# fgcallari/skeres

Hardware: AMD Instinct MI355X
Metric: LM iterations/sec (higher is better)
Workload: dtype f64

## Files before the change

### skeres_amd/csrc/chol_kernels.hip

```cpp
#include <hip/hip_runtime.h>
#include <algorithm>
#include <atomic>
#include <chrono>
#include <hip/hip_ext.h>
#include <math.h>
#include <stdlib.h>
#include <string.h>
#include <memory>
#include "chol_kernels.hpp"
#include "device_table.hpp"

namespace sk {

typedef double d4 __attribute__((ext_vector_type(4)));

constexpr int gemm_lds_doubles(int kBKT, int kTM, int kTN) { return 2 * (kTM + kTN) * (kBKT + 2); }
#define SK_GEMM_LDS(kBKT, kTM, kTN) __shared__ __attribute__((aligned(16))) double sh[gemm_lds_doubles(kBKT, kTM, kTN)];
template <int kMode, int kShape, int kBKT, int kPF, int kTM, int kTN>
__device__ __forceinline__ void gemm_nt_f64_body(double* shp, double* C, long ldc, const double* A, long lda, const double* B, long ldb, int K,
                                                 int tiles_m, int skip, int main_t = 0x7fffffff, int jump_t = 0, int main_n = 0x7fffffff,
                                                 int jump_n = 0, int block_id = -1, int* first_column_done = nullptr, int count_cols = 1,
                                                 int* diag_done = nullptr) {
  constexpr int mode = kMode;
  constexpr int kLdT = kBKT + 2;
// ... 85 lines not shown
  if (kPF == 2) { SK_LOAD_STAGE(1, (nk > 1 ? 1 : 0) * kBKT) }
  SK_STORE_STAGE(0, 0)
  __syncthreads();
#define SK_LOAD_STAGE_X(set, kbase) SK_LOAD_STAGE(set, kbase)
#define SK_STORE_STAGE_X(set, buf) SK_STORE_STAGE(set, buf)
#define SK_KSTEP(kt, SETL, SETS)                                                                   \
  {                                                                                                \
    const int buf = (kt) & 1;                                                                      \
    const int knext = ((kt) + kPF < nk ? (kt) + kPF : nk - 1) * kBKT;                              \
    SK_LOAD_STAGE_X(SETL, knext)                                                                   \
    const double* sa = &shp[buf * kShBuf + (wr * (kTM / 2) + l15) * kLdT + l4];                               \
    const double* sb = &shp[buf * kShBuf + (kTM + wc * (kTN / 2) + l15) * kLdT + l4];                         \
    _Pragma("unroll") for (int kk = 0; kk < kBKT / 4; ++kk) {                                      \
      double a[kMT], b[kNT];                                                                       \
      _Pragma("unroll") for (int m = 0; m < kMT; ++m) a[m] = sa[m * 16 * kLdT + kk * 4];           \
      _Pragma("unroll") for (int m = 0; m < kNT; ++m) b[m] = sb[m * 16 * kLdT + kk * 4];           \
      _Pragma("unroll") for (int mt = 0; mt < kMT; ++mt)                                           \
        _Pragma("unroll") for (int nt = 0; nt < kNT; ++nt)                                         \
          acc[mt][nt] = __builtin_amdgcn_mfma_f64_16x16x4f64(a[mt], b[nt], acc[mt][nt], 0, 0, 0);  \
    }                                                                                              \
    SK_STORE_STAGE_X(SETS, buf ^ 1)                                                                \
    __syncthreads();                                                                               \
  }
  if (kPF == 1) {
    for (int kt = 0; kt < nk; ++kt) SK_KSTEP(kt, 0, 0)
  } else {
    for (int kt = 0; kt < nk; kt += 2) {
      SK_KSTEP(kt, 0, 1)
      SK_KSTEP(kt + 1, 1, 0)
    }
  }
#undef SK_KSTEP
#undef SK_LOAD_STAGE_X
#undef SK_STORE_STAGE_X
  (void)ra1; (void)rb1;
#undef SK_LOAD_STAGE
#undef SK_STORE_STAGE
  const double sgn = mode == 0 ? -1.0 : 1.0;
  if (kShape == 2 && first_column_done && first_column) {
#pragma unroll
    for (int mt = 0; mt < kMT; ++mt)
#pragma unroll
      for (int nt = 0; nt < kNT; ++nt)
#pragma unroll
        for (int i = 0; i < 4; ++i)
          __hip_atomic_store(&Cg[(long)(crow + mt * 16 + 4 * i) * ldc + ccol + nt * 16], sgn * acc[mt][nt][i], __ATOMIC_RELAXED, __HIP_MEMORY_SCOPE_AGENT);
    asm volatile("s_waitcnt vmcnt(0) lgkmcnt(0)" ::: "memory");
    __syncthreads();
    if (threadIdx.x == 0) {
      __hip_atomic_fetch_add(first_column_done, 1, __ATOMIC_RELAXED, __HIP_MEMORY_SCOPE_AGENT);
      if (diag_done && diag_tile) __hip_atomic_fetch_add(diag_done, 16 / (128 / kTM), __ATOMIC_RELAXED, __HIP_MEMORY_SCOPE_AGENT);
    }
    return;
  }
#pragma unroll
  for (int mt = 0; mt < kMT; ++mt)
#pragma unroll
    for (int nt = 0; nt < kNT; ++nt)
#pragma unroll
      for (int i = 0; i < 4; ++i)
        Cg[(long)(crow + mt * 16 + 4 * i) * ldc + ccol + nt * 16] = sgn * acc[mt][nt][i];
}

__global__ __launch_bounds__(256, 2) void syrk_trailing_f64_kernel(double* C, long ldc, const double* A, long lda, int K, int tile_off, int main_t,
                                                                   int jump_t) {
  SK_GEMM_LDS(16, 128, 128)
  gemm_nt_f64_body<0, 1, 16, 1, 128, 128>(sh, C, ldc, A, lda, A, lda, K, 0, tile_off, main_t, jump_t);
}
__global__ __launch_bounds__(256, 2) void syrk_trailing_thin_f64_kernel(double* C, long ldc, const double* A, long lda, int K, int tiles_m, int main_t,
                                                                        int jump_t, int main_n, int jump_n, int* first_column_done, int count_cols, int* diag_done) {
  SK_GEMM_LDS(16, 32, 128)
  gemm_nt_f64_body<0, 2, 16, 2, 32, 128>(sh, C, ldc, A, lda, A, lda, K, tiles_m, 0, main_t, jump_t, main_n, jump_n, -1, first_column_done, count_cols, diag_done);
}
struct ThinSyrkArgs { double* C; long ldc; const double* A; long lda; int K, tiles_m, main_t, jump_t, main_n, jump_n; int* first_column_done; int grid; };
struct ThinSyrkPair { ThinSyrkArgs f[2]; };
__global__ __launch_bounds__(256, 2) void syrk_trailing_thin_pair_f64_kernel(ThinSyrkPair pair) {
  const ThinSyrkArgs& p = pair.f[blockIdx.y];
  if ((int)blockIdx.x >= p.grid) return;
  SK_GEMM_LDS(16, 32, 128)
  gemm_nt_f64_body<0, 2, 16, 2, 32, 128>(sh, p.C, p.ldc, p.A, p.lda, p.A, p.lda, p.K, p.tiles_m, 0, p.main_t, p.jump_t, p.main_n, p.jump_n, -1, p.first_column_done, 1, nullptr);
}
__global__ __launch_bounds__(256, 2) void syrk_gram_f64_kernel(double* C, long ldc, size_t slab_stride, const double* A, long lda, int K) {
  SK_GEMM_LDS(16, 128, 128)
  gemm_nt_f64_body<1, 1, 16, 1, 128, 128>(sh, C + (size_t)blockIdx.y * slab_stride, ldc, A + (size_t)blockIdx.y * K, lda, A + (size_t)blockIdx.y * K, lda, K, 0, 0);
}
__global__ __launch_bounds__(256) void gram_reduce_kernel(double* __restrict__ H, const double* __restrict__ slabs, size_t slab_stride, long ld,
                                                          int nslabs) {
  const int b = blockIdx.x;
  int r = (int)((sqrt(8.0 * (double)b + 1.0) - 1.0) * 0.5);
  while ((r + 1) * (r + 2) / 2 <= b) ++r;
  while (r * (r + 1) / 2 > b) --r;
  const int ti = r, tj = b - r * (r + 1) / 2;
  for (int e = threadIdx.x; e < 128 * 128; e += 256) {
    const size_t off = (size_t)(ti * 128 + (e >> 7)) * ld + tj * 128 + (e & 127);
    double s = 0.0;
    for (int c = 0; c < nslabs; ++c) s += slabs[(size_t)c * slab_stride + off];
    H[off] = s;
  }
}
__global__ __launch_bounds__(256, 2) void gemm_update_f64_kernel(double* C, long ldc, const double* A, long lda, const double* B,
                                                                 long ldb, int K, int tiles_m, int skip, int main_t, int jump_t) {
  __builtin_amdgcn_s_setprio(2);
  SK_GEMM_LDS(16, 64, 128)
  gemm_nt_f64_body<0, 0, 16, 2, 64, 128>(sh, C, ldc, A, lda, B, ldb, K, tiles_m, skip, main_t, jump_t);
}
__global__ __launch_bounds__(256, 2) void gemm_update_thin_f64_kernel(double* C, long ldc, const double* A, long lda, const double* B,
                                                                      long ldb, int K, int tiles_m, int skip, int main_t, int jump_t) {
  __builtin_amdgcn_s_setprio(2);
  SK_GEMM_LDS(16, 32, 128)
  gemm_nt_f64_body<0, 0, 16, 2, 32, 128>(sh, C, ldc, A, lda, B, ldb, K, tiles_m, skip, main_t, jump_t);
}
__global__ __launch_bounds__(256, 2) void trsm_gemm_thin_f64_kernel(double* C, long ldc, const double* A, long lda, const double* Linv,
                                                                    int tiles_m, int main_t, int jump_t) {
  __builtin_amdgcn_s_setprio(2);
  SK_GEMM_LDS(16, 32, 128)
  gemm_nt_f64_body<1, 0, 16, 2, 32, 128>(sh, C, ldc, A, lda, Linv, 128, 128, tiles_m, 0, main_t, jump_t);
}
__global__ __launch_bounds__(256, 1) void gemm_diag_f64_kernel(double* C, long ldc, const double* A, long lda, int K) {
  __builtin_amdgcn_s_setprio(3);
  SK_GEMM_LDS(32, 64, 64)
  gemm_nt_f64_body<0, 0, 32, 2, 64, 64>(sh, C, ldc, A, lda, A, lda, K, 2, 4);
}
__global__ __launch_bounds__(256, 2) void trsm_gemm_f64_kernel(double* C, long ldc, const double* A, long lda, const double* Linv,
                                                               int tiles_m, int main_t, int jump_t) {
  __builtin_amdgcn_s_setprio(2);
  SK_GEMM_LDS(16, 64, 128)
  gemm_nt_f64_body<1, 0, 16, 2, 64, 128>(sh, C, ldc, A, lda, Linv, 128, 128, tiles_m, 0, main_t, jump_t);
}

static constexpr int kB = 32, kBs = 33;
static constexpr int kBlk = kB * kBs;
__device__ __forceinline__ int blk_off(int bi, int bj) { return (bi * (bi + 1) / 2 + bj) * kBlk; }
__device__ __forceinline__ int inv_off(int bi, int bj) { return (10 + bi * (bi - 1) / 2 + bj) * kBlk; }

__device__ __forceinline__ double fast_rsqrt(double x) {
  double y = __builtin_amdgcn_rsq(x);
  double h = 0.5 * x;
  y = y * (1.5 - h * y * y);
  y = y * (1.5 - h * y * y);
  return y;
}
__device__ __forceinline__ double fast_rcp(double x) {
  const double y = __builtin_amdgcn_rcp(x);
  const double e = __builtin_fma(-x, y, 1.0);
  const double q = __builtin_fma(e, e, e);
  return __builtin_fma(y, q, y);
}
__device__ __forceinline__ double lane_bcast(double x, int src) {
  const int lo = __builtin_amdgcn_readlane(__double2loint(x), src);
  const int hi = __builtin_amdgcn_readlane(__double2hiint(x), src);
  return __hiloint2double(hi, lo);
}

__device__ __forceinline__ bool wave_potrf32(const double* D, double* colbuf, double (&a)[32], int lane) {
  const int row = lane & 31;
  const bool unit = lane >= 32;
#pragma unroll
  for (int c = 0; c < 32; ++c) {
    const double d = D[row * kBs + c];
    a[c] = unit ? (c == row ? 1.0 : 0.0) : d;
  }
  colbuf[lane] = a[0];
  typedef __attribute__((address_space(3))) const double* lds_cdp;
  unsigned cb_base = (unsigned)(unsigned long)(lds_cdp)colbuf;
  asm volatile("" : "+v"(cb_base));
  const lds_cdp cb3 = (lds_cdp)(unsigned long)cb_base;
  double cbp[32], cbn[32];
  double m_prev = 0.0, d_prev = 1.0;
  int dv_lo = 0, dv_hi = 0x3ff00000;
  int sgn = 0;
#define SK_PIN(x) asm volatile("" : "+v"(x));
#ifndef SK_PROBE_VARIANT
#define SK_PROBE_VARIANT 0
#endif
#define SK_FILL(k)                                                                                  \
  if (j >= 1 && SK_PROBE_VARIANT != 1) {                                                                                     \
    _Pragma("unroll") for (int c = j + 1 + ((k) * (31 - j) + 4) / 5; c < j + 1 + (((k) + 1) * (31 - j) + 4) / 5; ++c)  \
      a[c] = __builtin_fma(-m_prev, cbp[c], a[c]);                                                  \
  }
#pragma unroll
  for (int j = 0; j < 32; ++j) {
    {
      const lds_cdp cbj = cb3 + (j % 3) * 64;
#pragma unroll
      for (int c = j + 2; c < 32; ++c) cbn[c] = SK_PROBE_VARIANT == 2 ? a[c] * 0.5 : cbj[c];
    }
    const int d_lo = __builtin_amdgcn_readlane(__double2loint(a[j]), j), d_hi = __builtin_amdgcn_readlane(__double2hiint(a[j]), j);
    const double d = __hiloint2double(d_hi, d_lo);
    const double y = __builtin_amdgcn_rcp(d);
    const double l1 = lane_bcast(a[j], j + 1 < 32 ? j + 1 : j);
    const double m0 = a[j] * y;
    __builtin_amdgcn_sched_barrier(0);
    sgn |= d_hi;
    asm volatile("" : "+s"(sgn));
    asm volatile("v_writelane_b32 %0, %1, %2" : "+v"(dv_lo) : "s"(d_lo), "n"(j));
    asm volatile("v_writelane_b32 %0, %1, %2" : "+v"(dv_hi) : "s"(d_hi), "n"(j));
    SK_FILL(0)
    __builtin_amdgcn_sched_barrier(0);
    const double e = __builtin_fma(-d, y, 1.0);
    __builtin_amdgcn_sched_barrier(0);
    SK_FILL(1)
    __builtin_amdgcn_sched_barrier(0);
    const double q = __builtin_fma(e, e, e);
    __builtin_amdgcn_sched_barrier(0);
    SK_FILL(2)
    __builtin_amdgcn_sched_barrier(0);
    const double m = __builtin_fma(m0, q, m0);
    __builtin_amdgcn_sched_barrier(0);
    SK_FILL(3)
    __builtin_amdgcn_sched_barrier(0);
    if (j + 1 < 32) {
      a[j + 1] = __builtin_fma(-m, l1, a[j + 1]);
      colbuf[((j + 1) % 3) * 64 + lane] = a[j + 1];
    }
    __builtin_amdgcn_sched_barrier(0);
    SK_FILL(4)
    __builtin_amdgcn_sched_barrier(0);
    m_prev = m;
    d_prev = d;
#pragma unroll
    for (int c = j + 2; c < 32; ++c) cbp[c] = cbn[c];
  }
#undef SK_FILL
#undef SK_PIN
  {
    const double r = fast_rsqrt(__hiloint2double(dv_hi, dv_lo));
#pragma unroll
    for (int c = 0; c < 32; ++c) a[c] = a[c] * lane_bcast(r, c);
  }
  return sgn >= 0 && d_prev > 0.0;
}

template <bool kPlainB>
__device__ __forceinline__ void block_mma32(d4 (&acc)[2][2], const double* P, const double* Q, int lane) {
  const int l15 = lane & 15, l4 = lane >> 4;
#pragma unroll
  for (int kk = 0; kk < 8; ++kk) {
    const int k = kk * 4 + l4;
    double a[2], b[2];
#pragma unroll
    for (int m = 0; m < 2; ++m) {
      a[m] = P[(m * 16 + l15) * kBs + k];
      b[m] = kPlainB ? Q[k * kBs + m * 16 + l15] : Q[(m * 16 + l15) * kBs + k];
    }
#pragma unroll
    for (int mt = 0; mt < 2; ++mt)
#pragma unroll
      for (int nt = 0; nt < 2; ++nt)
        acc[mt][nt] = __builtin_amdgcn_mfma_f64_16x16x4f64(a[mt], b[nt], acc[mt][nt], 0, 0, 0);
  }
}
__device__ __forceinline__ void quad_mma16(d4& acc, const double* P, const double* Q, int qi, int qj, int lane, bool fresh) {
  const int l15 = lane & 15, l4 = lane >> 4;
  d4 a0 = fresh ? (d4){0.0, 0.0, 0.0, 0.0} : acc, a1 = (d4){0.0, 0.0, 0.0, 0.0};
#pragma unroll
  for (int kk = 0; kk < 8; kk += 2) {
    const int k = kk * 4 + l4;
    a0 = __builtin_amdgcn_mfma_f64_16x16x4f64(P[(qi * 16 + l15) * kBs + k], Q[(qj * 16 + l15) * kBs + k], a0, 0, 0, 0);
    a1 = __builtin_amdgcn_mfma_f64_16x16x4f64(P[(qi * 16 + l15) * kBs + k + 4], Q[(qj * 16 + l15) * kBs + k + 4], a1, 0, 0, 0);
  }
  acc = a0 + a1;
}
__device__ __forceinline__ void quad_store16(double* dst, const d4& acc, int qi, int qj, int lane, double sgn) {
  const int l15 = lane & 15, l4 = lane >> 4;
#pragma unroll
  for (int i = 0; i < 4; ++i) dst[(qi * 16 + l4 + 4 * i) * kBs + qj * 16 + l15] = sgn * acc[i];
}
__device__ __forceinline__ void quad_load16(d4& acc, const double* src, int qi, int qj, int lane, double sgn) {
  const int l15 = lane & 15, l4 = lane >> 4;
#pragma unroll
  for (int i = 0; i < 4; ++i) acc[i] = sgn * src[(qi * 16 + l4 + 4 * i) * kBs + qj * 16 + l15];
}
__device__ __forceinline__ void block_zero32(d4 (&acc)[2][2]) {
#pragma unroll
  for (int mt = 0; mt < 2; ++mt)
#pragma unroll
    for (int nt = 0; nt < 2; ++nt) acc[mt][nt] = (d4){0.0, 0.0, 0.0, 0.0};
}
__device__ __forceinline__ void block_store32(double* dst, const d4 (&acc)[2][2], int lane, double sgn) {
  const int l15 = lane & 15, l4 = lane >> 4;
#pragma unroll
  for (int mt = 0; mt < 2; ++mt)
#pragma unroll
    for (int nt = 0; nt < 2; ++nt)
#pragma unroll
      for (int i = 0; i < 4; ++i) dst[(mt * 16 + l4 + 4 * i) * kBs + nt * 16 + l15] = sgn * acc[mt][nt][i];
}
__device__ __forceinline__ void block_load32(d4 (&acc)[2][2], const double* src, int lane, double sgn) {
  const int l15 = lane & 15, l4 = lane >> 4;
#pragma unroll
  for (int mt = 0; mt < 2; ++mt)
#pragma unroll
    for (int nt = 0; nt < 2; ++nt)
#pragma unroll
      for (int i = 0; i < 4; ++i) acc[mt][nt][i] = sgn * src[(mt * 16 + l4 + 4 * i) * kBs + nt * 16 + l15];
}
__device__ __forceinline__ void block_update32(double* Cb, const double* P, const double* Q, int lane) {
  d4 acc[2][2];
  block_load32(acc, Cb, lane, -1.0);
  block_mma32<false>(acc, P, Q, lane);
  block_store32(Cb, acc, lane, -1.0);
}
__device__ __forceinline__ void block_to_global(double* dst, unsigned step2, unsigned goff, const double* src, int loff) {
#pragma unroll
  for (int i = 0; i < 16; ++i) dst[goff + i * step2] = src[loff + i * 2 * kBs];
}
__device__ __forceinline__ void block_neg_left_mul32(double* dst, const double* W, int lane) {
  d4 acc[2][2];
  block_zero32(acc);
  block_mma32<true>(acc, W, dst, lane);
  block_store32(dst, acc, lane, -1.0);
}

#ifdef SK_POTRF_STAMPS
__device__ long long g_potrf_stamps[4][16], g_potrf_clk[4][16];
#define SK_STAMP(i) if (lane == 0) { g_potrf_stamps[wave][i] = wall_clock64(); g_potrf_clk[wave][i] = clock64(); }
#else
#define SK_STAMP(i)
#endif

__device__ __forceinline__ void info_raise(int* info, int v) { (void)__hip_atomic_fetch_max(info, v, __ATOMIC_RELAXED, __HIP_MEMORY_SCOPE_AGENT); }

__device__ __forceinline__ void potrf128_body(double* lds_in, double* __restrict__ A, long ld, double* __restrict__ Linv, int* info) {
  double* lds = lds_in;
  int tid = threadIdx.x;
  asm volatile("" : "+v"(tid), "+s"(ld));
  double* T = lds;
  double* E = lds + 16 * kBlk;
  double* colbuf = lds + 18 * kBlk;
  volatile int* flags = reinterpret_cast<volatile int*>(colbuf + 192);
  const int t = tid, lane = t & 63, wave = __builtin_amdgcn_readfirstlane(t >> 6);
  __builtin_amdgcn_s_setprio(3);
  SK_STAMP(0)
  {
    double v0[4];
#pragma unroll
    for (int i = 0; i < 4; ++i) {
      const int e = t + 256 * i;
      v0[i] = A[(long)(e >> 5) * ld + (e & 31)];
    }
    if (wave == 0) {
#pragma unroll
      for (int i = 0; i < 4; ++i) { const int e = t + 256 * i; T[blk_off(0, 0) + (e >> 5) * kBs + (e & 31)] = v0[i]; }
      if (t < 4) flags[t] = 0;
      __syncthreads();
    } else {
      double v[3][16];
      const int first = 3 * (wave - 1) + 1;
      const long lo = (long)(lane >> 5) * ld + (lane & 31);
#pragma unroll
      for (int k = 0; k < 3; ++k) {
        const int idx = first + k, bi = idx >= 6 ? 3 : (idx >= 3 ? 2 : 1), bj = idx - bi * (bi + 1) / 2;
        const double* Ab = A + ((long)bi * kB * ld + bj * kB) + lo;
#pragma unroll
        for (int i = 0; i < 16; ++i) v[k][i] = Ab[(long)(2 * i) * ld];
      }
#pragma unroll
      for (int i = 0; i < 4; ++i) { const int e = t + 256 * i; T[blk_off(0, 0) + (e >> 5) * kBs + (e & 31)] = v0[i]; }
      __syncthreads();
      const int ll = (lane >> 5) * kBs + (lane & 31);
#pragma unroll
      for (int k = 0; k < 3; ++k) {
        const int idx = first + k, bi = idx >= 6 ? 3 : (idx >= 3 ? 2 : 1), bj = idx - bi * (bi + 1) / 2;
#pragma unroll
        for (int i = 0; i < 16; ++i) T[blk_off(bi, bj) + ll + 2 * i * kBs] = v[k][i];
      }
    }
  }
  SK_STAMP(1)
  const unsigned uld = (unsigned)ld;
  const unsigned go_a = (unsigned)(lane >> 5) * uld + (lane & 31), go_i = (unsigned)(lane >> 5) * 128u + (lane & 31);
  const int lo_w = (lane >> 5) * kBs + (lane & 31);
#define SK_L(bi, bj) (T + blk_off(bi, bj))
#define SK_V(bi, bj) (T + inv_off(bi, bj))
#define SK_GA(bi, bj) (A + ((long)(bi) * kB * ld + (bj) * kB))
#define SK_GI(bi, bj) (Linv + ((bi) * kB * 128 + (bj) * kB))
#define SK_PANEL_ROW(jb, bi)                                                                    \
  {                                                                                             \
    d4 acc[2][2];                                                                               \
    block_zero32(acc);                                                                          \
    block_mma32<false>(acc, SK_L(bi, jb), SK_L(jb, jb), lane);                                  \
    block_store32(SK_L(bi, jb), acc, lane, 1.0);   \
  }
#define SK_CRITICAL_B(jb)                                                                        \
  {                                                                                              \
    d4 xq;                                                                                       \
    quad_mma16(xq, SK_L((jb) + 1, jb), SK_L(jb, jb), qi, qj, lane, true);                        \
    __syncthreads();                                         \
    quad_store16(SK_L((jb) + 1, jb), xq, qi, qj, lane, 1.0);                                     \
    __syncthreads();                                                 \
    d4 uq;                                                                                       \
    quad_load16(uq, SK_L((jb) + 1, (jb) + 1), qi, qj, lane, -1.0);                               \
    quad_mma16(uq, SK_L((jb) + 1, jb), SK_L((jb) + 1, jb), qi, qj, lane, false);                 \
    quad_store16(SK_L((jb) + 1, (jb) + 1), uq, qi, qj, lane, -1.0);                              \
    __syncthreads();                                                                             \
  }
#define SK_WRITE_L(bi, bj) block_to_global(SK_GA(bi, bj), 2 * uld, go_a, SK_L(bi, bj), lo_w);
#define SK_WRITE_W(bi) block_to_global(SK_GI(bi, bi), 256u, go_i, SK_L(bi, bi), lo_w);
#define SK_WRITE_V(bi, bj) block_to_global(SK_GI(bi, bj), 256u, go_i, SK_V(bi, bj), lo_w);
#define SK_WRITE_E(bi) block_to_global(SK_GA(bi, bi), 2 * uld, go_a, E + ((bi) & 1) * kBlk, lo_w);
#define SK_FLAG_SET(i) { __builtin_amdgcn_fence(__ATOMIC_RELEASE, "workgroup"); __builtin_amdgcn_wave_barrier(); if (lane == 0) flags[i] = 1; }
#define SK_FLAG_WAIT(i) { while (__builtin_amdgcn_readfirstlane(flags[i]) == 0) __builtin_amdgcn_s_sleep(1); __builtin_amdgcn_fence(__ATOMIC_ACQUIRE, "workgroup"); }
  const int qi = wave >> 1, qj = wave & 1;
  if (wave == 0) {
#pragma unroll 1
    for (int jb = 0; jb < 4; ++jb) {
      double* D = SK_L(jb, jb);
      double a[32];
      const bool ok = wave_potrf32(D, colbuf, a, lane);
      SK_STAMP(11 + jb)
      if (!ok && lane == 0) info_raise(info, 1);
      {
        const int row = lane & 31;
        double* dst = lane < 32 ? E + (jb & 1) * kBlk + row * kBs : D + row;
        const int step = lane < 32 ? 1 : kBs;
#pragma unroll
        for (int c = 0; c < 32; ++c) dst[c * step] = a[c];
      }
      SK_STAMP(2 + 2 * jb)
      __syncthreads();
      if (jb == 0) SK_CRITICAL_B(0)
      if (jb == 1) SK_CRITICAL_B(1)
      if (jb == 2) SK_CRITICAL_B(2)
      SK_STAMP(3 + 2 * jb)
    }
  } else {
    d4 accs[2][2];
    SK_STAMP(2)
    __syncthreads();
    SK_CRITICAL_B(0)
    SK_STAMP(3)
    if (wave == 1) {
      SK_PANEL_ROW(0, 2)
      SK_FLAG_SET(0)
      block_update32(SK_L(2, 2), SK_L(2, 0), SK_L(2, 0), lane);
      block_update32(SK_L(2, 1), SK_L(2, 0), SK_L(1, 0), lane);
      SK_WRITE_L(2, 0)
    }
    if (wave == 2) {
      SK_PANEL_ROW(0, 3)
      SK_FLAG_SET(1)
      block_update32(SK_L(3, 3), SK_L(3, 0), SK_L(3, 0), lane);
      block_update32(SK_L(3, 1), SK_L(3, 0), SK_L(1, 0), lane);
      SK_WRITE_L(3, 0)
    }
    if (wave == 3) {
      SK_WRITE_E(0) SK_WRITE_L(1, 0) SK_WRITE_W(0)
      SK_FLAG_WAIT(0) SK_FLAG_WAIT(1)
      block_update32(SK_L(3, 2), SK_L(3, 0), SK_L(2, 0), lane);
    }
    SK_STAMP(4)
    __syncthreads();
    SK_CRITICAL_B(1)
    SK_STAMP(5)
    if (wave == 1) {
      SK_PANEL_ROW(1, 3)
      block_update32(SK_L(3, 3), SK_L(3, 1), SK_L(3, 1), lane);
      block_update32(SK_L(3, 2), SK_L(3, 1), SK_L(2, 1), lane);
      SK_WRITE_L(3, 1) SK_WRITE_L(2, 1)
    }
    if (wave == 2) {
      d4 acc[2][2];
      block_zero32(acc);
      block_mma32<true>(acc, SK_L(1, 0), SK_L(0, 0), lane);
      block_store32(SK_V(1, 0), acc, lane, 1.0);
      block_neg_left_mul32(SK_V(1, 0), SK_L(1, 1), lane);
      SK_FLAG_SET(2)
      block_zero32(acc);
      block_mma32<true>(acc, SK_L(2, 1), SK_L(1, 1), lane);
      block_store32(SK_V(2, 1), acc, lane, 1.0);
      SK_WRITE_V(1, 0)
    }
    if (wave == 3) {
      SK_WRITE_E(1) SK_WRITE_W(1)
      block_zero32(accs);
      block_mma32<true>(accs, SK_L(2, 0), SK_L(0, 0), lane);
      SK_FLAG_WAIT(2)
      block_mma32<true>(accs, SK_L(2, 1), SK_V(1, 0), lane);
      block_store32(SK_V(2, 0), accs, lane, 1.0);
    }
    SK_STAMP(6)
    __syncthreads();
    SK_CRITICAL_B(2)
    SK_STAMP(7)
    if (wave == 1) {
      block_zero32(accs);
      block_mma32<true>(accs, SK_L(3, 0), SK_L(0, 0), lane);
      block_mma32<true>(accs, SK_L(3, 1), SK_V(1, 0), lane);
      SK_WRITE_L(3, 2)
      SK_FLAG_WAIT(3)
      block_mma32<true>(accs, SK_L(3, 2), SK_V(2, 0), lane);
      block_store32(SK_V(3, 0), accs, lane, 1.0);
      SK_WRITE_V(2, 0)
    }
    if (wave == 2) {
      block_neg_left_mul32(SK_V(2, 1), SK_L(2, 2), lane);
      block_zero32(accs);
      block_mma32<true>(accs, SK_L(3, 1), SK_L(1, 1), lane);
      block_mma32<true>(accs, SK_L(3, 2), SK_V(2, 1), lane);
      block_store32(SK_V(3, 1), accs, lane, 1.0);
      SK_WRITE_V(2, 1)
    }
    if (wave == 3) {
      block_neg_left_mul32(SK_V(2, 0), SK_L(2, 2), lane);
      SK_FLAG_SET(3)
      block_zero32(accs);
      block_mma32<true>(accs, SK_L(3, 2), SK_L(2, 2), lane);
      block_store32(SK_V(3, 2), accs, lane, 1.0);
      SK_WRITE_E(2) SK_WRITE_W(2)
    }
    SK_STAMP(8)
    __syncthreads();
  }
  if (wave < 3) {
    block_neg_left_mul32(SK_V(3, wave), SK_L(3, 3), lane);
    SK_WRITE_V(3, wave)
  } else {
    SK_WRITE_E(3) SK_WRITE_W(3)
  }
  SK_STAMP(10)
#undef SK_PANEL_ROW
#undef SK_CRITICAL_B
#undef SK_FLAG_SET
#undef SK_FLAG_WAIT
#undef SK_WRITE_L
#undef SK_WRITE_W
#undef SK_WRITE_V
#undef SK_WRITE_E
#undef SK_L
#undef SK_V
#undef SK_GA
#undef SK_GI
}

__global__ __launch_bounds__(256, 1) void potrf128_kernel(double* __restrict__ A, long ld, double* __restrict__ Linv, int* info) {
  extern __shared__ __attribute__((aligned(16))) double lds[];
  potrf128_body(lds, A, ld, Linv, info);
}
enum : int { kSyncPotrfDone = 0, kSyncAbort = 1, kSyncSyrkSeq = 2, kSyncSyrkColumn = 3, kSyncServerXcc = 4, kSyncPotrfFast = 5, kSyncStart = 6, kSyncEnd = 7,
             kSyncXSlot = 16, kSyncDSlot = 32, kSyncHeader = 64 };
constexpr int kSyncArrays = 3;
constexpr int kCritCandidates = 160;
constexpr long long kChainTimeoutTicks = 100000000;

__device__ long long g_chain_stamps[1024][8];
__device__ int g_chain_stamps_on;
#define SK_CHAIN_STAMP(col, i) if (g_chain_stamps_on && threadIdx.x == 0 && (col) < 512) g_chain_stamps[(col) + 512 * stamp_front][i] = wall_clock64();
__device__ __forceinline__ int sync_load(const int* p) { return __hip_atomic_load(p, __ATOMIC_RELAXED, __HIP_MEMORY_SCOPE_AGENT); }
__device__ __forceinline__ bool chain_wait(const int* p, int target, int* abort_flag) {
  if (sync_load(p) < target) {
    const long long t0 = wall_clock64();
    do {
      __builtin_amdgcn_s_sleep(4);
      if (sync_load(abort_flag) != 0) return false;
      if (wall_clock64() - t0 > kChainTimeoutTicks) {
        __hip_atomic_store(abort_flag, 1, __ATOMIC_RELAXED, __HIP_MEMORY_SCOPE_AGENT);
        return false;
      }
    } while (sync_load(p) < target);
  }
  __builtin_amdgcn_fence(__ATOMIC_ACQUIRE, "agent");
  asm volatile("s_waitcnt vmcnt(0)" ::: "memory");
  return true;
}
__device__ __forceinline__ bool chain_wait_start(const int* p, int value) {
  if (sync_load(p) != value) {
    const long long t0 = wall_clock64();
    int spins = 0;
    do {
      __builtin_amdgcn_s_sleep(8);
      if ((++spins & 63) == 0 && wall_clock64() - t0 > 30 * kChainTimeoutTicks) return false;
    } while (sync_load(p) != value);
  }
  __builtin_amdgcn_fence(__ATOMIC_ACQUIRE, "agent");
  asm volatile("s_waitcnt vmcnt(0)" ::: "memory");
  return true;
}
#ifdef SK_CHAIN_STRONG_FENCES
#define SK_CHAIN_ACQUIRE_ALL __builtin_amdgcn_fence(__ATOMIC_ACQUIRE, "agent");
#else
#define SK_CHAIN_ACQUIRE_ALL
#endif
__device__ __forceinline__ void chain_publish(int* p, int add) {
#ifdef SK_CHAIN_STRONG_FENCES
  __builtin_amdgcn_fence(__ATOMIC_RELEASE, "agent");
  __syncthreads();
  if (threadIdx.x == 0) __hip_atomic_fetch_add(p, add, __ATOMIC_RELAXED, __HIP_MEMORY_SCOPE_AGENT);
#else
  asm volatile("s_waitcnt vmcnt(0) lgkmcnt(0)" ::: "memory");
  __syncthreads();
  if (threadIdx.x == 0) {
    __builtin_amdgcn_fence(__ATOMIC_RELEASE, "agent");
    __hip_atomic_fetch_add(p, add, __ATOMIC_RELAXED, __HIP_MEMORY_SCOPE_AGENT);
  }
#endif
}

__device__ __forceinline__ void store_through(double* p, double v) { __hip_atomic_store(p, v, __ATOMIC_RELAXED, __HIP_MEMORY_SCOPE_AGENT); }
__device__ __forceinline__ void chain_publish_through(int* p, int add) {
  asm volatile("s_waitcnt vmcnt(0) lgkmcnt(0)" ::: "memory");
  __syncthreads();
  if (threadIdx.x == 0) __hip_atomic_fetch_add(p, add, __ATOMIC_RELAXED, __HIP_MEMORY_SCOPE_AGENT);
}

typedef int int16v __attribute__((ext_vector_type(16)));
__device__ __forceinline__ int load_l2(const int* p) {
  int v;
  asm volatile("s_dcache_inv\n\ts_load_dword %0, %1, 0x0\n\ts_waitcnt lgkmcnt(0)" : "=s"(v) : "s"(p) : "memory");
  return v;
}
__device__ __forceinline__ int min16_l2(const int* p) {
  int16v v;
  asm volatile("s_dcache_inv\n\ts_load_dwordx16 %0, %1, 0x0\n\ts_waitcnt lgkmcnt(0)" : "=s"(v) : "s"(p) : "memory");
  int m = v[0];
#pragma unroll
  for (int i = 1; i < 16; ++i) m = v[i] < m ? v[i] : m;
  return m;
}
__device__ __forceinline__ int xcc_id() {
  int v;
  asm volatile("s_getreg_b32 %0, hwreg(HW_REG_XCC_ID)" : "=s"(v));
  return v & 0xf;
}
__device__ __forceinline__ void store_l2(int* p, int v) { *(volatile int*)p = v; }
__device__ __forceinline__ bool chain_wait_l2(const int* p, int target, int* abort_flag) {
  if (load_l2(p) < target) {
    const long long t0 = wall_clock64();
    int spins = 0;
    do {
      __builtin_amdgcn_s_sleep(2);
      if ((++spins & 63) == 0) {
        if (sync_load(abort_flag) != 0) return false;
        if (wall_clock64() - t0 > kChainTimeoutTicks) { __hip_atomic_store(abort_flag, 1, __ATOMIC_RELAXED, __HIP_MEMORY_SCOPE_AGENT); return false; }
      }
    } while (load_l2(p) < target);
  }
  return true;
}
__device__ __forceinline__ bool chain_wait_slots(const int* slots, int target, int* abort_flag) {
  if (min16_l2(slots) < target) {
    const long long t0 = wall_clock64();
    int spins = 0;
    do {
      __builtin_amdgcn_s_sleep(2);
      if ((++spins & 63) == 0) {
        if (sync_load(abort_flag) != 0) return false;
        if (wall_clock64() - t0 > kChainTimeoutTicks) { __hip_atomic_store(abort_flag, 1, __ATOMIC_RELAXED, __HIP_MEMORY_SCOPE_AGENT); return false; }
      }
    } while (min16_l2(slots) < target);
  }
  return true;
}
__device__ __forceinline__ bool server_wait_diag(int* sync, int j, int local) {
  const int* slots = sync + kSyncDSlot;
  const int* counter = sync + kSyncHeader + j;
  int* abort_flag = sync + kSyncAbort;
  if (!local) return chain_wait(counter, 16, abort_flag);
  const long long t0 = wall_clock64();
  for (int spins = 0;; ++spins) {
    if (min16_l2(slots) >= j) return true;
    if ((spins & 15) == 0) {
      if (sync_load(counter) >= 16) {
        __builtin_amdgcn_fence(__ATOMIC_ACQUIRE, "agent");
        asm volatile("s_waitcnt vmcnt(0)" ::: "memory");
        return true;
      }
      if (sync_load(abort_flag) != 0) return false;
      if (wall_clock64() - t0 > kChainTimeoutTicks) { __hip_atomic_store(abort_flag, 1, __ATOMIC_RELAXED, __HIP_MEMORY_SCOPE_AGENT); return false; }
    }
    __builtin_amdgcn_s_sleep(2);
  }
// ... 407 lines not shown
        if (jn == 0 && g_bs_test_janitor_giveup && atomicExch(&g_bs_test_janitor_giveup, 0) != 0) ok = 0;
#endif
        if (!ok && info) info_raise(info, 2);
        ok_s = ok;
      }
      __syncthreads();
      if (!ok_s) return;
      const int top = min((int)env.top[kb], nblk - 1);
      const int tlo = max((int)env.tail[kb], top + 1);
      double* col = S + (long)(rg * 16) * ld + (long)kb * 128 + c;
      int visited = 0;
      for (int cur = kb + 1; cur < nblk; ++cur) {
        if (cur > top && cur < tlo) { cur = tlo - 1; continue; }
        if ((visited++) % parts != part) continue;
        double* pz = col + (long)cur * 128 * ld;
#pragma unroll
        for (int i = 0; i < 16; ++i) pz[(long)i * ld] = 0.0;
      }
      __syncthreads();
    }
    return;
  }
  __shared__ double ysh[128], wsh[128], part[16][128];
  __shared__ int abort_s;
  const int kb = nown - 1 - block;
  const int t = threadIdx.x, c = t & 127, rg = t >> 7;
  if (t == 0) abort_s = 0;
  if (t < 128) { const int j = kb * 128 + t; wsh[t] = j < n ? rhs[j] : 0.0; }
  double li[16], lr[16];
  {
    const double* p = Linv + (long)kb * 128 * 128 + (long)(rg * 16) * 128 + c;
#pragma unroll
    for (int i = 0; i < 16; ++i) li[i] = p[(long)i * 128];
  }
  const int top = min((int)env.top[kb], nblk - 1);
  const int tlo = max((int)env.tail[kb], top + 1);
  int cur = (kb < nblk - 1 && tlo <= nblk - 1) ? nblk - 1 : top;
  const double* Lcol = S + (long)(rg * 16) * ld + (long)kb * 128 + c;
  if (cur > kb) {
    const double* p = Lcol + (long)cur * 128 * ld;
#pragma unroll
    for (int i = 0; i < 16; ++i) lr[i] = p[(long)i * ld];
  }
  __syncthreads();
  while (cur > kb) {
    if (g_bs_stamps_on && t == 0 && cur == kb + 1) g_bs_stamps[kb][0] = wall_clock64();
    if (t < 128 && cur >= nown) {
      const int bi = (cur - nown) * 128 + t;
      const int src = yb_map ? yb_map[bi] : bi;
      ysh[t] = src >= 0 ? yb[src] : 0.0;
    } else if (t < 128) {
      const unsigned long long* src = reinterpret_cast<const unsigned long long*>(y + (long)cur * 128 + t);
      unsigned long long v = a.l2_poll ? load_sc0_u64(src) : __hip_atomic_load(src, __ATOMIC_RELAXED, __HIP_MEMORY_SCOPE_AGENT);
      if (v == kBsSentinel) {
        const long long t0 = wall_clock64();
        int spins = 0;
        do {
          __builtin_amdgcn_s_sleep(1);
          if (a.l2_poll) {
            v = load_sc0_u64(src);
            if (v == kBsSentinel && (++spins & 3) == 0) v = __hip_atomic_load(src, __ATOMIC_RELAXED, __HIP_MEMORY_SCOPE_AGENT);
          } else {
            v = __hip_atomic_load(src, __ATOMIC_RELAXED, __HIP_MEMORY_SCOPE_AGENT);
          }
          if (v == kBsSentinel && wall_clock64() - t0 > kChainTimeoutTicks) { abort_s = 1; v = 0ull; }
        } while (v == kBsSentinel);
      }
      ysh[t] = __longlong_as_double((long long)v);
    }
    __syncthreads();
    if (g_bs_stamps_on && t == 0 && cur == kb + 1) g_bs_stamps[kb][1] = wall_clock64();
#pragma unroll
    for (int g = 0; g < 2; ++g) {
      double sacc = 0.0;
#pragma unroll
      for (int i = 0; i < 8; ++i) sacc += lr[g * 8 + i] * ysh[rg * 16 + g * 8 + i];
      part[rg * 2 + g][c] = sacc;
    }
    const int nxt = (cur > top && cur - 1 < tlo) ? top : cur - 1;
    if (nxt > kb) {
      const double* p = Lcol + (long)nxt * 128 * ld;
#pragma unroll
      for (int i = 0; i < 16; ++i) lr[i] = p[(long)i * ld];
    }

    __syncthreads();
    if (t < 128) {
      double u = 0.0;
#pragma unroll
      for (int g = 0; g < 16; ++g) u += part[g][t];
      wsh[t] -= u;
    }
    cur = nxt;
  }
  __syncthreads();
  {
    double sacc = 0.0;
#pragma unroll
    for (int i = 0; i < 16; ++i) sacc += li[i] * wsh[rg * 16 + i];
    part[rg][c] = sacc;
  }
  __syncthreads();
  if (t < 128) {
    double sacc = 0.0;
#pragma unroll
    for (int q = 0; q < 8; ++q) sacc += part[q][t];
    unsigned long long bits = (unsigned long long)__double_as_longlong(sacc);
    if (bits == kBsSentinel) bits ^= 1ull;
    if (a.l2_poll) *reinterpret_cast<volatile unsigned long long*>(y + (long)kb * 128 + t) = bits;
    __hip_atomic_store(reinterpret_cast<unsigned long long*>(y + (long)kb * 128 + t), bits, __ATOMIC_RELAXED, __HIP_MEMORY_SCOPE_AGENT);
    if (g_bs_stamps_on && t == 0) { asm volatile("s_waitcnt vmcnt(0)" ::: "memory"); g_bs_stamps[kb][2] = wall_clock64(); }
  }
  if (t == 0 && abort_s && info) info_raise(info, 2);
}

__global__ __launch_bounds__(1024, 1) void bs_resident_kernel(const double* __restrict__ Linv, double* S, long ld, const double* rhs,
                                                               int n, double* y, int nblk, BsTop env, int* info, int nown, const double* __restrict__ yb, int zero_after ,
                                                               const int* __restrict__ yb_map) {
  const int spread = zero_after < 0 ? 1 : 0;
  const BsArgs a{Linv, S, ld, rhs, n, y, nblk, info, nown, yb, spread ? 7 * nown : zero_after, yb_map, spread ? 7 : 0, spread};
  const int b = (int)blockIdx.x;
  bs_resident_body(a, env, spread ? ((b & 7) == 0 ? b >> 3 : nown + (b >> 3) * 7 + (b & 7) - 1) : b);
}
constexpr int kBsPairMaxBlocks = 448;
struct BsTopHalf { unsigned short top[kBsPairMaxBlocks]; unsigned short tail[kBsPairMaxBlocks]; };
struct BsPair { BsArgs f[2]; BsTopHalf env[2]; };
__global__ __launch_bounds__(1024, 1) void bs_resident_pair_kernel(BsPair p) {
  const int b = (int)blockIdx.x, nA = p.f[0].nown, nB = p.f[1].nown, own = nA + nB;
  int front, blk;
  if (p.f[0].jan_parts > 0) {
    const int g = b >> 3, slot = b & 7;
    front = slot >> 2;
    const int nown = front ? nB : nA;
    if (g >= nown) return;
    blk = (slot & 3) == 0 ? g : nown + g * 3 + (slot & 3) - 1;
    bs_resident_body(p.f[front], p.env[front], blk);
    return;
  }
  if (b < own) {
    const int m = nA < nB ? nA : nB;
    if (b < 2 * m) { front = b & 1; blk = b >> 1; } else { front = nA > nB ? 0 : 1; blk = b - m; }
  } else {
    const int j = b - own;
    if (j < p.f[0].janitors) { front = 0; blk = nA + j; } else { front = 1; blk = nB + (j - p.f[0].janitors); }
  }
  bs_resident_body(p.f[front], p.env[front], blk);
}

__global__ void copy_row_kernel(const double* __restrict__ src, double* __restrict__ dst, int n, int npad) {
  const int j = blockIdx.x * blockDim.x + threadIdx.x;
  if (j < npad) dst[j] = j < n ? src[j] : 0.0;
}

static const size_t g_potrf_lds = (size_t)(18 * kBlk + 192 + 4) * sizeof(double);
size_t potrf128_lds_bytes() { return g_potrf_lds; }

static std::vector<hipStream_t> g_orphan_streams;
constexpr int g_early_column = 1;
constexpr int g_thin_grid = 512;
constexpr int g_ext_events = 1;
constexpr unsigned g_event_flags = hipEventDisableTiming | hipEventDisableSystemFence;
static int g_chain_server = 1;
constexpr int g_chain_max_trailing = 24, g_chain_prefix_group = 2;
static int g_pair_max_trailing = 0;
constexpr int g_thin_syrk_tiles = 48;
constexpr int g_tail_tiles = 48, g_tail_group = 1;
static int g_chain_local = 0;
static std::atomic<int> g_bs_resident{1};
#ifdef SK_TESTING
static std::atomic<int> g_test_withhold{-1};
static std::atomic<int> g_test_janitor_giveup{0};
#endif
hipError_t cholesky_init() {
  static std::once_flag once;
  std::call_once(once, [] {
#ifdef SK_TESTING
    if (const char* e = getenv("SK_CHAIN_TEST_WITHHOLD_MARKER")) g_test_withhold.store(atoi(e));
    if (const char* e = getenv("SK_BS_TEST_JANITOR_GIVEUP")) g_test_janitor_giveup.store(atoi(e) > 0 ? 1 : 0);
#endif
    const DevKnobs& k = dev_knobs();
    g_bs_resident.store(k.bs_resident);
    g_chain_server = k.chain_server;
    g_pair_max_trailing = k.pair_max_trailing;
    g_chain_local = k.chain_xcd_local;
  });
  hipError_t rc = hipFuncSetAttribute(reinterpret_cast<const void*>(potrf_server_kernel), hipFuncAttributeMaxDynamicSharedMemorySize, (int)g_potrf_lds);
  if (rc != hipSuccess) return rc;
  rc = hipFuncSetAttribute(reinterpret_cast<const void*>(potrf_server_pair_kernel), hipFuncAttributeMaxDynamicSharedMemorySize, (int)g_potrf_lds);
  if (rc != hipSuccess) return rc;
  return hipFuncSetAttribute(reinterpret_cast<const void*>(potrf128_kernel), hipFuncAttributeMaxDynamicSharedMemorySize, 160 * 1024);
}

CholeskyContext::~CholeskyContext() {
  for (hipEvent_t e : events) (void)hipEventDestroy(e);
  if (fork_ev) (void)hipEventDestroy(fork_ev);
  if (join_ev) (void)hipEventDestroy(join_ev);
  if (sync) (void)hipFree(sync);
  if (xs) (void)hipFree(xs);
}

int* CholeskyContext::sync_for(int nblk) {
  if (nblk > sync_blk) {
    if (sync) (void)hipFree(sync);
    if (xs) (void)hipFree(xs);
    sync = nullptr; xs = nullptr;
    sync_blk = 0;
    const int cap = (nblk + 63) / 64 * 64;
    if (hipMalloc(reinterpret_cast<void**>(&xs), sizeof(double) * 128 * 128 * (size_t)cap) != hipSuccess) { (void)hipGetLastError(); xs = nullptr; return nullptr; }
    if (hipMalloc(reinterpret_cast<void**>(&sync), sizeof(int) * (size_t)(kSyncHeader + kSyncArrays * cap)) != hipSuccess) { (void)hipGetLastError(); sync = nullptr; return nullptr; }
    sync_blk = cap;
  }
  return sync;
}

constexpr int kBulkCand = 2, kPanelCand = 4, kServerCand = 3;
struct DeviceQueues {
  int device = -1;
  hipStream_t panel = nullptr, bulk = nullptr, bulk_early = nullptr, server = nullptr;
  int reserved_cus = 0, early_tiles = 0;
  hipStream_t bulk_candidates[kBulkCand] = {}, bulk_early_candidates[kBulkCand] = {}, panel_candidates[kPanelCand] = {},
              server_candidates[kServerCand] = {};
  std::vector<hipStream_t> all_streams;
  int queue_choice = -1;
  std::atomic<bool> tuning{false};
  std::atomic<int> chain_server{1};
  std::atomic<int> pair_users{0};
  hipStream_t fork = nullptr;
  hipStream_t plain[2] = {nullptr, nullptr};
  std::mutex enqueue_mutex[2];
};
static PerDeviceTable<DeviceQueues> g_device_queues;

static hipError_t create_bulk_stream(hipStream_t* out, int per_xcd, int ncu, int* reserved) {
  *reserved = 0;
  if (per_xcd > 0 && ncu >= 64 && ncu % 8 == 0 && per_xcd < ncu / 8) {
    std::vector<uint32_t> mask((size_t)(ncu + 31) / 32, 0u);
    for (int i = per_xcd * 8; i < ncu; ++i) mask[(size_t)i / 32] |= 1u << (i % 32);
    if (hipExtStreamCreateWithCUMask(out, (uint32_t)mask.size(), mask.data()) == hipSuccess) { *reserved = per_xcd * 8; return hipSuccess; }
    (void)hipGetLastError();
  }
  return hipStreamCreateWithFlags(out, hipStreamNonBlocking);
}

static DeviceQueues* create_device_queues(int dev) {
  std::unique_ptr<DeviceQueues> q(new DeviceQueues());
  q->device = dev;
  q->chain_server.store(g_chain_server);
  int ncu = 0, reserved = 0, reserved_early = 0;
  (void)hipDeviceGetAttribute(&ncu, hipDeviceAttributeMultiprocessorCount, dev);
  const int per_xcd = dev_knobs().bulk_reserve >= 0 ? dev_knobs().bulk_reserve : 4, per_xcd_early = dev_knobs().bulk_reserve_early >= 0 ? dev_knobs().bulk_reserve_early : 2, early_tiles = 72;
  if (dev_knobs().queue_shift > 0) {
    std::vector<uint32_t> all((size_t)(ncu + 31) / 32, 0xffffffffu);
    for (int k = 0; k < dev_knobs().queue_shift; ++k) {
      hipStream_t d = nullptr;
      if (hipExtStreamCreateWithCUMask(&d, (uint32_t)all.size(), all.data()) != hipSuccess) (void)hipGetLastError();
      else q->all_streams.push_back(d);
    }
  }
  auto fail = [&]() -> DeviceQueues* {
    for (hipStream_t st : q->all_streams) g_orphan_streams.push_back(st);
    return nullptr;
  };
  hipStream_t b = nullptr, be = nullptr;
  if (create_bulk_stream(&b, per_xcd, ncu, &reserved) != hipSuccess) { (void)hipGetLastError(); return fail(); }
  q->all_streams.push_back(b);
  if (create_bulk_stream(&be, per_xcd_early, ncu, &reserved_early) != hipSuccess) { (void)hipGetLastError(); return fail(); }
  q->all_streams.push_back(be);
  q->bulk_candidates[0] = b; q->bulk_early_candidates[0] = be;
  hipStream_t p = nullptr, sv = nullptr;
  if (reserved > 0) {
    const size_t words = (size_t)(ncu + 31) / 32;
    std::vector<uint32_t> cu0(words, 0u), rest(words, 0u);
    cu0[0] = 0xffu;
    for (int i = 8; i < ncu; ++i) rest[(size_t)i / 32] |= 1u << (i % 32);
    bool ok = true;
    auto masked = [&](hipStream_t* out, const std::vector<uint32_t>& m) {
      if (!ok) return;
      if (hipExtStreamCreateWithCUMask(out, (uint32_t)words, m.data()) != hipSuccess) { (void)hipGetLastError(); *out = nullptr; ok = false; return; }
      q->all_streams.push_back(*out);
    };
    for (int k = 1; k < kBulkCand && ok; ++k) {
      int r = 0;
      if (create_bulk_stream(&q->bulk_candidates[k], per_xcd, ncu, &r) != hipSuccess || create_bulk_stream(&q->bulk_early_candidates[k], per_xcd_early, ncu, &r) != hipSuccess) {
        (void)hipGetLastError();
        ok = false;
      }
      if (q->bulk_candidates[k]) q->all_streams.push_back(q->bulk_candidates[k]);
      if (q->bulk_early_candidates[k]) q->all_streams.push_back(q->bulk_early_candidates[k]);
    }
    for (int k = 0; k < kPanelCand; ++k) masked(&q->panel_candidates[k], rest);
    for (int k = 0; k < kServerCand; ++k) masked(&q->server_candidates[k], cu0);
    p = q->panel_candidates[0];
    sv = p ? q->server_candidates[0] : nullptr;
    if (!ok) q->queue_choice = 0;
    if (dev_knobs().chain_queues >= 0) q->queue_choice = dev_knobs().chain_queues % (kBulkCand * kPanelCand * kServerCand);
    if (ok && q->queue_choice >= 0) {
      b = q->bulk_candidates[q->queue_choice / (kPanelCand * kServerCand)];
      be = q->bulk_early_candidates[q->queue_choice / (kPanelCand * kServerCand)];
      p = q->panel_candidates[q->queue_choice / kServerCand % kPanelCand];
      sv = q->server_candidates[q->queue_choice % kServerCand];
    }
  }
  if (!p) {
    if (hipStreamCreateWithFlags(&p, hipStreamNonBlocking) != hipSuccess) { (void)hipGetLastError(); return fail(); }
    q->all_streams.push_back(p);
  }
  q->server = sv; q->panel = p; q->bulk = b; q->bulk_early = be; q->reserved_cus = reserved; q->early_tiles = early_tiles;
// ... 991 lines not shown
```

Baseline: 260.4.

## Skip zero triangular MFMA blocks and restructure wave potrf column publishing

```diff
diff --git a/skeres_amd/csrc/chol_kernels.hip b/skeres_amd/csrc/chol_kernels.hip
--- a/skeres_amd/csrc/chol_kernels.hip
+++ b/skeres_amd/csrc/chol_kernels.hip
@@ -261,7 +261,16 @@
   return __hiloint2double(hi, lo);
 }
 
-__device__ __forceinline__ bool wave_potrf32(const double* D, double* colbuf, double (&a)[32], int lane) {
+#ifdef SK_POTRF_STAMPS
+__device__ long long g_potrf_stamps[4][24], g_potrf_clk[4][24];
+#define SK_STAMP(i) if (lane == 0) { g_potrf_stamps[wave][i] = wall_clock64(); g_potrf_clk[wave][i] = clock64(); }
+#else
+#define SK_STAMP(i)
+#endif
+
+__device__ __forceinline__ bool wave_potrf32(const double* D, double* pub, double (&a)[32], int lane, int jb) {
+  constexpr int wave = 0;
+  (void)wave; (void)jb;
   const int row = lane & 31;
   const bool unit = lane >= 32;
 #pragma unroll
@@ -269,42 +278,49 @@
     const double d = D[row * kBs + c];
     a[c] = unit ? (c == row ? 1.0 : 0.0) : d;
   }
-  colbuf[lane] = a[0];
   typedef __attribute__((address_space(3))) const double* lds_cdp;
-  unsigned cb_base = (unsigned)(unsigned long)(lds_cdp)colbuf;
-  asm volatile("" : "+v"(cb_base));
+  typedef __attribute__((address_space(3))) double* lds_dp;
+  unsigned cb_base = (unsigned)(unsigned long)(lds_cdp)pub;
+  unsigned my_base = cb_base + 8u * (unsigned)(lane < 32 ? lane : 32);
+  asm volatile("" : "+v"(cb_base), "+v"(my_base));
   const lds_cdp cb3 = (lds_cdp)(unsigned long)cb_base;
+  const lds_dp mine = (lds_dp)(unsigned long)my_base;
+  mine[0] = a[0];
   double cbp[32], cbn[32];
-  double m_prev = 0.0, d_prev = 1.0;
-  int dv_lo = 0, dv_hi = 0x3ff00000;
-  int sgn = 0;
+  double m_prev = 0.0;
+  unsigned cb_row = cb_base;
 #define SK_PIN(x) asm volatile("" : "+v"(x));
 #ifndef SK_PROBE_VARIANT
 #define SK_PROBE_VARIANT 0
 #endif
-#define SK_FILL(k)                                                                                  \
-  if (j >= 1 && SK_PROBE_VARIANT != 1) {                                                                                     \
-    _Pragma("unroll") for (int c = j + 1 + ((k) * (31 - j) + 4) / 5; c < j + 1 + (((k) + 1) * (31 - j) + 4) / 5; ++c)  \
-      a[c] = __builtin_fma(-m_prev, cbp[c], a[c]);                                                  \
-  }
+#define SK_FILL_RANGE(lo, hi)                                                                       \
+  if (j >= 1 && SK_PROBE_VARIANT != 1) {                                                            \
+    _Pragma("unroll") for (int c = (lo); c < (hi); ++c) a[c] = __builtin_fma(-m_prev, cbp[c], a[c]); \
+  }
+#define SK_FILL_LO(k) (j + 1 + ((k) * (31 - j) + 4) / 5)
+#define SK_FILL(k) SK_FILL_RANGE(SK_FILL_LO(k), SK_FILL_LO((k) + 1))
 #pragma unroll
   for (int j = 0; j < 32; ++j) {
     {
-      const lds_cdp cbj = cb3 + (j % 3) * 64;
+      if (j % 7 == 0) {
+        cb_row = cb_base + (unsigned)(j * kBs * sizeof(double));
+        asm volatile("" : "+v"(cb_row));
+      }
+      const lds_cdp cbj = (lds_cdp)(unsigned long)cb_row + (j % 7) * kBs;
 #pragma unroll
       for (int c = j + 2; c < 32; ++c) cbn[c] = SK_PROBE_VARIANT == 2 ? a[c] * 0.5 : cbj[c];
     }
-    const int d_lo = __builtin_amdgcn_readlane(__double2loint(a[j]), j), d_hi = __builtin_amdgcn_readlane(__double2hiint(a[j]), j);
-    const double d = __hiloint2double(d_hi, d_lo);
+    const double d = lane_bcast(a[j], j);
+    __builtin_amdgcn_sched_barrier(0);
+    const double l1 = lane_bcast(a[j], j + 1 < 32 ? j + 1 : j);
+    __builtin_amdgcn_sched_barrier(0);
     const double y = __builtin_amdgcn_rcp(d);
-    const double l1 = lane_bcast(a[j], j + 1 < 32 ? j + 1 : j);
+    __builtin_amdgcn_sched_barrier(0);
+    SK_FILL_RANGE(j + 1, j + 2 < 32 ? j + 2 : 32)
+    __builtin_amdgcn_sched_barrier(0);
     const double m0 = a[j] * y;
     __builtin_amdgcn_sched_barrier(0);
-    sgn |= d_hi;
-    asm volatile("" : "+s"(sgn));
-    asm volatile("v_writelane_b32 %0, %1, %2" : "+v"(dv_lo) : "s"(d_lo), "n"(j));
-    asm volatile("v_writelane_b32 %0, %1, %2" : "+v"(dv_hi) : "s"(d_hi), "n"(j));
-    SK_FILL(0)
+    SK_FILL_RANGE(j + 2, SK_FILL_LO(1))
     __builtin_amdgcn_sched_barrier(0);
     const double e = __builtin_fma(-d, y, 1.0);
     __builtin_amdgcn_sched_barrier(0);
@@ -320,27 +336,31 @@
     __builtin_amdgcn_sched_barrier(0);
     if (j + 1 < 32) {
       a[j + 1] = __builtin_fma(-m, l1, a[j + 1]);
-      colbuf[((j + 1) % 3) * 64 + lane] = a[j + 1];
+      mine[(j + 1) * kBs] = a[j + 1];
     }
     __builtin_amdgcn_sched_barrier(0);
     SK_FILL(4)
     __builtin_amdgcn_sched_barrier(0);
     m_prev = m;
-    d_prev = d;
 #pragma unroll
     for (int c = j + 2; c < 32; ++c) cbp[c] = cbn[c];
   }
 #undef SK_FILL
+#undef SK_FILL_LO
+#undef SK_FILL_RANGE
 #undef SK_PIN
+  SK_STAMP(16 + jb)
+  const double dl = cb3[row * (kBs + 1)];
   {
-    const double r = fast_rsqrt(__hiloint2double(dv_hi, dv_lo));
-#pragma unroll
-    for (int c = 0; c < 32; ++c) a[c] = a[c] * lane_bcast(r, c);
-  }
-  return sgn >= 0 && d_prev > 0.0;
-}
-
-template <bool kPlainB>
+    const double r = fast_rsqrt(dl);
+    ((lds_dp)(unsigned long)cb_base)[row] = r;
+#pragma unroll
+    for (int c = 0; c < 32; ++c) a[c] = a[c] * cb3[c];
+  }
+  return __builtin_amdgcn_ballot_w64(!(dl > 0.0 && dl < __builtin_inf())) == 0;
+}
+
+template <bool kPlainB, int kTri = 0>
 __device__ __forceinline__ void block_mma32(d4 (&acc)[2][2], const double* P, const double* Q, int lane) {
   const int l15 = lane & 15, l4 = lane >> 4;
 #pragma unroll
@@ -355,8 +375,12 @@
 #pragma unroll
     for (int mt = 0; mt < 2; ++mt)
 #pragma unroll
-      for (int nt = 0; nt < 2; ++nt)
+      for (int nt = 0; nt < 2; ++nt) {
+        if (kTri == 1 && !kPlainB && nt == 0 && kk >= 4) continue;
+        if (kTri == 1 && kPlainB && nt == 1 && kk < 4) continue;
+        if (kTri == 2 && mt == 0 && kk >= 4) continue;
         acc[mt][nt] = __builtin_amdgcn_mfma_f64_16x16x4f64(a[mt], b[nt], acc[mt][nt], 0, 0, 0);
+      }
   }
 }
 __device__ __forceinline__ void quad_mma16(d4& acc, const double* P, const double* Q, int qi, int qj, int lane, bool fresh) {
@@ -417,16 +441,9 @@
 __device__ __forceinline__ void block_neg_left_mul32(double* dst, const double* W, int lane) {
   d4 acc[2][2];
   block_zero32(acc);
-  block_mma32<true>(acc, W, dst, lane);
+  block_mma32<true, 2>(acc, W, dst, lane);
   block_store32(dst, acc, lane, -1.0);
 }
-
-#ifdef SK_POTRF_STAMPS
-__device__ long long g_potrf_stamps[4][16], g_potrf_clk[4][16];
-#define SK_STAMP(i) if (lane == 0) { g_potrf_stamps[wave][i] = wall_clock64(); g_potrf_clk[wave][i] = clock64(); }
-#else
-#define SK_STAMP(i)
-#endif
 
 __device__ __forceinline__ void info_raise(int* info, int v) { (void)__hip_atomic_fetch_max(info, v, __ATOMIC_RELAXED, __HIP_MEMORY_SCOPE_AGENT); }
 
@@ -436,8 +453,8 @@
   asm volatile("" : "+v"(tid), "+s"(ld));
   double* T = lds;
   double* E = lds + 16 * kBlk;
-  double* colbuf = lds + 18 * kBlk;
-  volatile int* flags = reinterpret_cast<volatile int*>(colbuf + 192);
+  double* pub = lds + 18 * kBlk;
+  volatile int* flags = reinterpret_cast<volatile int*>(pub + kBlk);
   const int t = tid, lane = t & 63, wave = __builtin_amdgcn_readfirstlane(t >> 6);
   __builtin_amdgcn_s_setprio(3);
   SK_STAMP(0)
@@ -488,7 +505,7 @@
   {                                                                                             \
     d4 acc[2][2];                                                                               \
     block_zero32(acc);                                                                          \
-    block_mma32<false>(acc, SK_L(bi, jb), SK_L(jb, jb), lane);                                  \
+    block_mma32<false, 1>(acc, SK_L(bi, jb), SK_L(jb, jb), lane);         \
     block_store32(SK_L(bi, jb), acc, lane, 1.0);   \
   }
 #define SK_CRITICAL_B(jb)                                                                        \
@@ -516,7 +533,7 @@
     for (int jb = 0; jb < 4; ++jb) {
       double* D = SK_L(jb, jb);
       double a[32];
-      const bool ok = wave_potrf32(D, colbuf, a, lane);
+      const bool ok = wave_potrf32(D, pub, a, lane, jb);
       SK_STAMP(11 + jb)
       if (!ok && lane == 0) info_raise(info, 1);
       {
@@ -571,19 +588,19 @@
     if (wave == 2) {
       d4 acc[2][2];
       block_zero32(acc);
-      block_mma32<true>(acc, SK_L(1, 0), SK_L(0, 0), lane);
+      block_mma32<true, 1>(acc, SK_L(1, 0), SK_L(0, 0), lane);
       block_store32(SK_V(1, 0), acc, lane, 1.0);
       block_neg_left_mul32(SK_V(1, 0), SK_L(1, 1), lane);
       SK_FLAG_SET(2)
       block_zero32(acc);
-      block_mma32<true>(acc, SK_L(2, 1), SK_L(1, 1), lane);
+      block_mma32<true, 1>(acc, SK_L(2, 1), SK_L(1, 1), lane);
       block_store32(SK_V(2, 1), acc, lane, 1.0);
       SK_WRITE_V(1, 0)
     }
     if (wave == 3) {
       SK_WRITE_E(1) SK_WRITE_W(1)
       block_zero32(accs);
-      block_mma32<true>(accs, SK_L(2, 0), SK_L(0, 0), lane);
+      block_mma32<true, 1>(accs, SK_L(2, 0), SK_L(0, 0), lane);
       SK_FLAG_WAIT(2)
       block_mma32<true>(accs, SK_L(2, 1), SK_V(1, 0), lane);
       block_store32(SK_V(2, 0), accs, lane, 1.0);
@@ -594,7 +611,7 @@
     SK_STAMP(7)
     if (wave == 1) {
       block_zero32(accs);
-      block_mma32<true>(accs, SK_L(3, 0), SK_L(0, 0), lane);
+      block_mma32<true, 1>(accs, SK_L(3, 0), SK_L(0, 0), lane);
       block_mma32<true>(accs, SK_L(3, 1), SK_V(1, 0), lane);
       SK_WRITE_L(3, 2)
       SK_FLAG_WAIT(3)
@@ -605,7 +622,7 @@
     if (wave == 2) {
       block_neg_left_mul32(SK_V(2, 1), SK_L(2, 2), lane);
       block_zero32(accs);
-      block_mma32<true>(accs, SK_L(3, 1), SK_L(1, 1), lane);
+      block_mma32<true, 1>(accs, SK_L(3, 1), SK_L(1, 1), lane);
       block_mma32<true>(accs, SK_L(3, 2), SK_V(2, 1), lane);
       block_store32(SK_V(3, 1), accs, lane, 1.0);
       SK_WRITE_V(2, 1)
@@ -614,18 +631,54 @@
       block_neg_left_mul32(SK_V(2, 0), SK_L(2, 2), lane);
       SK_FLAG_SET(3)
       block_zero32(accs);
-      block_mma32<true>(accs, SK_L(3, 2), SK_L(2, 2), lane);
+      block_mma32<true, 1>(accs, SK_L(3, 2), SK_L(2, 2), lane);
       block_store32(SK_V(3, 2), accs, lane, 1.0);
       SK_WRITE_E(2) SK_WRITE_W(2)
     }
     SK_STAMP(8)
     __syncthreads();
   }
-  if (wave < 3) {
-    block_neg_left_mul32(SK_V(3, wave), SK_L(3, 3), lane);
-    SK_WRITE_V(3, wave)
-  } else {
-    SK_WRITE_E(3) SK_WRITE_W(3)
+  {
+    const int l15 = lane & 15, l4 = lane >> 4;
+    const double* W3 = SK_L(3, 3);
+    d4 q[3];
+#pragma unroll
+    for (int i = 0; i < 3; ++i) q[i] = (d4){0.0, 0.0, 0.0, 0.0};
+    SK_STAMP(9)
+    if (wave < 3) {
+      const double* S3 = SK_V(3, wave);
+#pragma unroll
+      for (int kk = 0; kk < 8; ++kk) {
+        const int k = kk * 4 + l4;
+        const double a1 = W3[(16 + l15) * kBs + k], b0 = S3[k * kBs + l15], b1 = S3[k * kBs + 16 + l15];
+        if (kk < 4) q[0] = __builtin_amdgcn_mfma_f64_16x16x4f64(W3[l15 * kBs + k], b0, q[0], 0, 0, 0);
+        q[1] = __builtin_amdgcn_mfma_f64_16x16x4f64(a1, b0, q[1], 0, 0, 0);
+        q[2] = __builtin_amdgcn_mfma_f64_16x16x4f64(a1, b1, q[2], 0, 0, 0);
+      }
+      double* G = SK_GI(3, wave) + l4 * 128 + l15;
+#pragma unroll
+      for (int i = 0; i < 4; ++i) {
+        G[(4 * i) * 128] = -q[0][i];
+        G[(16 + 4 * i) * 128] = -q[1][i];
+        G[(16 + 4 * i) * 128 + 16] = -q[2][i];
+      }
+      SK_STAMP(15)
+    } else {
+#pragma unroll
+      for (int kk = 0; kk < 4; ++kk) {
+        const int k = kk * 4 + l4;
+        const double a0 = W3[l15 * kBs + k];
+#pragma unroll
+        for (int bj = 0; bj < 3; ++bj) q[bj] = __builtin_amdgcn_mfma_f64_16x16x4f64(a0, SK_V(3, bj)[k * kBs + 16 + l15], q[bj], 0, 0, 0);
+      }
+      double* G = SK_GI(3, 0) + l4 * 128 + 16 + l15;
+#pragma unroll
+      for (int i = 0; i < 4; ++i)
+#pragma unroll
+        for (int bj = 0; bj < 3; ++bj) G[(4 * i) * 128 + bj * kB] = -q[bj][i];
+      SK_STAMP(15)
+      SK_WRITE_E(3) SK_WRITE_W(3)
+    }
   }
   SK_STAMP(10)
 #undef SK_PANEL_ROW
@@ -1339,7 +1392,7 @@
   if (j < npad) dst[j] = j < n ? src[j] : 0.0;
 }
 
-static const size_t g_potrf_lds = (size_t)(18 * kBlk + 192 + 4) * sizeof(double);
+static const size_t g_potrf_lds = (size_t)(19 * kBlk + 4) * sizeof(double);
 size_t potrf128_lds_bytes() { return g_potrf_lds; }
 
 static std::vector<hipStream_t> g_orphan_streams;
```

Result: no change. 260.7 (median of 3 runs) (+0.1%).
